# MasterXiong/Hyper-VLA

Measured on AMD Instinct MI355X. Metric: actions_per_sec, higher is better.
Workload: dtype f16; 1 GPU; BASELINE configs[1]: hypernet weight-gen once (untimed) + full sample_actions step (u8 224x224 -> DINOv2-base E=768 in the loop -> generated vit_t 4L/64d policy -> [4,7] action chunk); 1 action = 1 sample-step; batch_per_gpu=256, global_batch=256, encoder=DINOv2-base (reference parity, E=768), parallelism=episode-dp1 (no collectives), policy_operands=split-bf16 (bf16x3), launch=eager (114 launches per step, counted by the library), streams=1, ensemble=not in the step

## Files before the change

### hyper-vla_amd/csrc/api.hip

```cpp
#include <hip/hip_runtime.h>

#include <cmath>
#include <cstdio>
#include <cstring>
#include <map>
#include <memory>
#include <mutex>
#include <string>
#include <vector>

#include "../../include/hvla.h"
#include "common.h"
#include "kernels.h"
#include "layout.h"
#include "pack.h"
#include "serving_layout.h"
#include "t5.h"
#include "train.h"

using namespace hvla;

namespace {

struct DevBuf {
// ... 1058 lines not shown
  return HVLA_OK;
}

int hvla_profile_read(hvla_ctx* ctx, float* ms, int32_t* launches) {
  if (!ctx || !ms || !launches) return HVLA_E_STATE;
  HIPCHK(ctx, hipSetDevice(ctx->device));
  for (int i = 0; i < HVLA_PROF_N; ++i) ms[i] = 0.f, launches[i] = 0;
  Profiler& p = ctx->prof;
  for (size_t i = 0; i < p.used; ++i) {
    HIPCHK(ctx, hipEventSynchronize(p.stop[i]));
    float t = 0.f;
    HIPCHK(ctx, hipEventElapsedTime(&t, p.start[i], p.stop[i]));
    ms[p.cat[i]] += t;
    launches[p.cat[i]] += 1;
  }
  p.used = 0;
  return HVLA_OK;
}

#ifdef HVLA_BENCH_HOOKS
int hvla_debug_gemm(hvla_ctx* ctx, int M, int N, int K, int epi, int variant, int iters, float* ms) {
  if (!ctx || !ctx->loaded) return HVLA_E_STATE;
  HIPCHK(ctx, hipSetDevice(ctx->device));
  const void* A = ctx->ws[K > ctx->g.E ? WS_G : WS_H].p;
  void* out = ctx->ws[epi == 3 ? WS_X : (epi == 1 ? WS_QKV : WS_G)].p;
  if (epi == 2 && K > ctx->g.E) return HVLA_E_SHAPE;
  const EncLayerW& L = ctx->encw.layer[0];
  const void* W = epi == 1 ? L.wqkv : (epi == 2 ? L.w1 : (K > ctx->g.E ? L.w2 : L.wo));
  const float* bias = epi == 1 ? L.bqkv : (epi == 2 ? L.b1 : L.b2);
  HIPCHK(ctx, debug_gemm(A, W, bias, L.ls1, out, M, N, K, epi, variant, iters, ms, nullptr));
  return HVLA_OK;
}

int hvla_debug_bgemm(const float* A, const float* B, float* C, int M, int N, int K, int ta, int tb, int nb, int accumulate,
                     int iters, float* ms) {
  const int lda = ta ? M : K, ldb = tb ? K : N;
  BG g{A, B, C, nullptr, M, N, K, lda, ldb, N, (long)M * K, 0, (long)N * K, 0, (long)M * N, 0, 0, 1, 1.f, accumulate, 1, accumulate != 0};
  hipEvent_t e0, e1;
  (void)hipEventCreate(&e0);
  (void)hipEventCreate(&e1);
  for (int i = 0; i < 3; ++i) bgemm(nullptr, ta != 0, tb != 0, g, nb);
  (void)hipEventRecord(e0, nullptr);
  for (int i = 0; i < iters; ++i) bgemm(nullptr, ta != 0, tb != 0, g, nb);
  (void)hipEventRecord(e1, nullptr);
  (void)hipEventSynchronize(e1);
  (void)hipEventElapsedTime(ms, e0, e1);
  *ms /= iters;
  (void)hipEventDestroy(e0);
  (void)hipEventDestroy(e1);
  return hipGetLastError() == hipSuccess ? HVLA_OK : HVLA_E_HIP;
}

struct hvla_bgemm_desc {
  const float* A;
  const float* B;
  float* C;
  const float* bias;
  int32_t M, N, K, lda, ldb, ldc;
  int64_t sA0, sA1, sB0, sB1, sC0, sC1, sBias0, sBias1;
  int32_t nb1;
  float alpha;
  int32_t accumulate, ksplit, allow_split, a_padded;
  int32_t ta, tb, nb0;
};
int hvla_debug_bgemm_once(const hvla_bgemm_desc* d, int32_t* chosen) {
  if (!d || !chosen || d->nb0 < 1 || d->nb1 < 1 || d->ksplit < 1 || d->M < 1 || d->N < 1 || d->K < 1) return (int)hipErrorInvalidValue;
// ... 110 lines not shown
```

### hyper-vla_amd/csrc/encoder.hip

```cpp
#include <cstring>
#include <type_traits>

#include "common.h"
#include "kernels.h"
#include "plan.h"

namespace hvla {

template <typename Op>
__global__ void im2col_kernel(const uint8_t* __restrict__ img, typename Op::elem* __restrict__ out, int B,
                              int image, int patch, int grid, int Kp, float* __restrict__ x, const float* __restrict__ pos, int S, int E) {
  for (size_t i = (size_t)blockIdx.x * blockDim.x + threadIdx.x; i < (size_t)B * E; i += (size_t)gridDim.x * blockDim.x)
    x[(i / E) * S * E + (i % E)] = pos[i % E];
  const int Kp1 = Kp / 2, chunks = Kp1 / 8;
  const size_t total = (size_t)B * grid * grid * chunks;
  const int kreal = patch * patch * 3;
  for (size_t i = (size_t)blockIdx.x * blockDim.x + threadIdx.x; i < total; i += (size_t)gridDim.x * blockDim.x) {
    const int ch = (int)(i % chunks);
    const size_t m = i / chunks;
    const int px = (int)(m % grid), py = (int)((m / grid) % grid);
    const size_t b = m / ((size_t)grid * grid);
    typename Op::x8 v;
    const int rowb = 3 * patch;
    const int k0 = ch * 8;
// ... 25 lines not shown
  const void* abar2 = nullptr;
  const void* dW2 = nullptr;
  float* corr2 = nullptr;
  int M2 = 0;
  int row0 = 0, row_step = 1;
  int hsplit = 1 << 30;
  int tile_row0 = 0, tile_stride = 256, nbm = 0;
  void* colmean = nullptr;
  void* ln_out = nullptr;
  const float* ln_scale = nullptr;
  const float* ln_bias = nullptr;
  void* ln_abar = nullptr;
  uint32_t* ln_cnt = nullptr;
  float* ln_part = nullptr;
  uint32_t ln_target = 0;
  uint32_t ln_tag = 0;
  uint32_t ln_spin = 0;
  uint32_t out_bytes = 0;
  uint32_t part_bytes = 0;
  int lnx_G = 0, lnx_rows_aligned = 0, lnx_rounds_div = 0, lnx_rows_xcd = 0, lnx_rcp = 0;
  const float* ln_partial = nullptr;
};

__device__ __forceinline__ int wperm(int rho) { return (rho & ~63) + 4 * (rho & 15) + ((rho >> 4) & 3); }
__device__ __forceinline__ f32x4 corr_value(f32x4 acc, float b) {
  return f32x4{fmaf(acc[0], 1.f / 4096.f, b), fmaf(acc[1], 1.f / 4096.f, b), fmaf(acc[2], 1.f / 4096.f, b), fmaf(acc[3], 1.f / 4096.f, b)};
}

template <typename Op, int EPI, int MT, bool FULL, bool ROWBIAS, bool CS = false, bool WT = false, bool NT = false>
__device__ __forceinline__ void gemm_epilogue_rows_impl(const f32x4 (&acc)[4][MT], const GemmArgs& g, int m_base, int n_base,
                                                        int fr, int fq, const f32x4* pre_b4, const f32x4* pre_l4,
                                                        typename Op::x4* cs = nullptr,
                                                        const __attribute__((address_space(3))) float* lds_corr = nullptr,
                                                        int lds_img0 = -1) {
  using T = typename Op::elem;
  const int n = n_base + 4 * fr;
  f32x4 b4 = f32x4{0.f, 0.f, 0.f, 0.f};
  if constexpr (!ROWBIAS) b4 = pre_b4 ? *pre_b4 : *reinterpret_cast<const f32x4*>(g.bias + n);
  f32x4 l4 = f32x4{1.f, 1.f, 1.f, 1.f};
  if constexpr (EPI == EPI_RES) l4 = pre_l4 ? *pre_l4 : *reinterpret_cast<const f32x4*>(g.aux + n);
  const float q = EPI == EPI_PATCH ? g.qscale : ((EPI == EPI_QKV && n_base < g.qcols) ? g.qscale : 1.f);
  __amdgpu_buffer_rsrc_t wt_rsrc;
  if constexpr (WT) wt_rsrc = __builtin_amdgcn_make_buffer_rsrc(g.out, 0, (int)g.out_bytes, 0x00020000);
  auto store_f32x4 = [&](uint32_t elem_off, f32x4 v) {
    if constexpr (WT) __builtin_amdgcn_raw_buffer_store_b128(__builtin_bit_cast(u32x4, v), wt_rsrc, (int)(elem_off * 4u), 0, 16);
    else *reinterpret_cast<f32x4*>(reinterpret_cast<float*>(g.out) + elem_off) = v;
  };
  __amdgpu_buffer_rsrc_t nt_rsrc;
  uint32_t nt_vo = 0;
  if constexpr (NT && FULL && (EPI == EPI_QKV || EPI == EPI_GELU)) {
    nt_rsrc = __builtin_amdgcn_make_buffer_rsrc(g.out, 0, -1, 0x00020000);
    nt_vo = ((uint32_t)(g.row0 + (m_base + 4 * fq) * g.row_step) * (uint32_t)g.N + (uint32_t)n) * (uint32_t)sizeof(T);
  }
  constexpr int RB = MT < 2 ? 1 : (EPI == EPI_RES && MT >= 4 ? 4 : 2);
#pragma unroll
  for (int mp = 0; mp < MT; mp += RB) {
    f32x4 xin[RB][4], brow[RB][4];
    uint32_t off[RB][4];
    bool ok[RB][4];
#pragma unroll
    for (int u = 0; u < RB; ++u)
#pragma unroll
      for (int r = 0; r < 4; ++r) {
        const int m = m_base + (mp + u) * 16 + 4 * fq + r;
        ok[u][r] = FULL || m < g.M;
        const int grow = g.row0 + m * g.row_step;
        off[u][r] = (uint32_t)grow * (uint32_t)g.N + (uint32_t)n;
        if constexpr (EPI == EPI_PATCH) {
          const int prow = 1 + (m % g.P);
          off[u][r] = (uint32_t)((m / g.P) * g.S + prow) * (uint32_t)g.N + (uint32_t)n;
          if (ok[u][r]) xin[u][r] = *reinterpret_cast<const f32x4*>(g.aux + (uint32_t)prow * (uint32_t)g.N + (uint32_t)n);
        }
        if constexpr (EPI == EPI_RES) {
          if (ok[u][r]) {
            if constexpr (NT) xin[u][r] = __builtin_nontemporal_load(reinterpret_cast<const f32x4*>(reinterpret_cast<const float*>(g.out) + off[u][r]));
            else xin[u][r] = *reinterpret_cast<const f32x4*>(reinterpret_cast<const float*>(g.out) + off[u][r]);
          }
        }
        if constexpr (ROWBIAS) {
          brow[u][r] = f32x4{0.f, 0.f, 0.f, 0.f};
          const int img = grow / g.S;
          const int tok = grow - img * g.S, hf = tok >= g.hsplit ? 1 : 0;
          if (lds_img0 >= 0) {
            if (ok[u][r]) {
              if (tok) brow[u][r] = *reinterpret_cast<const __attribute__((address_space(3))) f32x4*>(lds_corr + ((img - lds_img0) * 2 + hf) * 64 + 4 * fr);
              else brow[u][r] = *reinterpret_cast<const f32x4*>(g.bias + (uint32_t)n);
            }
          } else {
            const float* bsrc = tok ? g.corr + (uint32_t)(img * 2 + hf) * (uint32_t)g.N : g.bias;
            if (ok[u][r]) brow[u][r] = *reinterpret_cast<const f32x4*>(bsrc + (uint32_t)n);
          }
        }
      }
#pragma unroll
    for (int u = 0; u < RB; ++u) {
      f32x4 t[4];
#pragma unroll
      for (int c = 0; c < 4; ++c) {
        if constexpr (EPI == EPI_PATCH) t[c] = __builtin_elementwise_fma(acc[c][mp + u], f32x4{q, q, q, q}, f32x4{b4[c], b4[c], b4[c], b4[c]});
        else if constexpr (EPI == EPI_CORR) t[c] = corr_value(acc[c][mp + u], b4[c]);
        else if constexpr (ROWBIAS) t[c] = acc[c][mp + u] + f32x4{brow[u][0][c], brow[u][1][c], brow[u][2][c], brow[u][3][c]};
        else t[c] = acc[c][mp + u] + b4[c];
        if constexpr (EPI == EPI_QKV) t[c] *= q;
        if constexpr (EPI == EPI_GELU) {
          const f32x2 g0 = gelu_erf2(f32x2{t[c][0], t[c][1]}), g1 = gelu_erf2(f32x2{t[c][2], t[c][3]});
          t[c] = f32x4{g0[0], g0[1], g1[0], g1[1]};
        }
// ... 2 lines not shown
      for (int r = 0; r < 4; ++r) {
        if (!ok[u][r]) continue;
        if constexpr (EPI == EPI_QKV || EPI == EPI_GELU) {
          typename Op::x4 o;
#pragma unroll
          for (int c = 0; c < 4; ++c) o[c] = (T)t[c][r];
          if constexpr (CS) *cs += o;
          if constexpr (NT && FULL) {
            int rowb = g.row_step * g.N * (int)sizeof(T);
            asm volatile("" : "+s"(rowb));
            __builtin_amdgcn_raw_buffer_store_b64(__builtin_bit_cast(u32x2, o), nt_rsrc, (int)nt_vo, ((mp + u) * 16 + r) * rowb, 2);
          } else if constexpr (NT) __builtin_nontemporal_store(o, reinterpret_cast<typename Op::x4*>(reinterpret_cast<T*>(g.out) + off[u][r]));
          else *reinterpret_cast<typename Op::x4*>(reinterpret_cast<T*>(g.out) + off[u][r]) = o;
        } else if constexpr (EPI == EPI_RES) {
          f32x4 x = xin[u][r];
#pragma unroll
          for (int c = 0; c < 4; ++c) x[c] = fmaf(t[c][r], l4[c], x[c]);
          store_f32x4(off[u][r], x);
        } else if constexpr (EPI == EPI_CORR) {
          *reinterpret_cast<f32x4*>(reinterpret_cast<float*>(g.out) + off[u][r]) = f32x4{t[0][r], t[1][r], t[2][r], t[3][r]};
        } else {
          f32x4 x = xin[u][r];
#pragma unroll
          for (int c = 0; c < 4; ++c) x[c] += t[c][r];
          store_f32x4(off[u][r], x);
        }
      }
    }
  }
}

template <typename Op, int EPI, int MT>
__device__ __forceinline__ void gemm_epilogue_rows(const f32x4 (&acc)[4][MT], const GemmArgs& g, int m_base, int n_base,
                                                   int fr, int fq) {
  const bool full = m_base + 16 * MT <= g.M;
  if constexpr (EPI == EPI_PATCH || EPI == EPI_CORR) {
    if (full) gemm_epilogue_rows_impl<Op, EPI, MT, true, false>(acc, g, m_base, n_base, fr, fq, nullptr, nullptr);
    else gemm_epilogue_rows_impl<Op, EPI, MT, false, false>(acc, g, m_base, n_base, fr, fq, nullptr, nullptr);
  } else {
    if (g.corr) {
      if (full) gemm_epilogue_rows_impl<Op, EPI, MT, true, true>(acc, g, m_base, n_base, fr, fq, nullptr, nullptr);
      else gemm_epilogue_rows_impl<Op, EPI, MT, false, true>(acc, g, m_base, n_base, fr, fq, nullptr, nullptr);
    } else {
      if (full) gemm_epilogue_rows_impl<Op, EPI, MT, true, false>(acc, g, m_base, n_base, fr, fq, nullptr, nullptr);
      else gemm_epilogue_rows_impl<Op, EPI, MT, false, false>(acc, g, m_base, n_base, fr, fq, nullptr, nullptr);
    }
  }
}


template <typename Op, int EPI>
__global__ __launch_bounds__(256, 2) void gemm_kernel(GemmArgs g) {
  using T = typename Op::elem;
  using X8 = typename Op::x8;
  extern __shared__ __attribute__((aligned(16))) char smem[];
  T* As = reinterpret_cast<T*>(smem);
  T* Ws = As + 2 * GBM * GLD;
  const int tid = threadIdx.x, wave = tid >> 6, lane = tid & 63;
  const int wm = wave >> 1, wn = wave & 1;
  const int nbm = (g.M + GBM - 1) / GBM, nbn = g.N / GBN;
  const int bid = xcd_run(blockIdx.x, nbm * nbn);
  const int bm = bid % nbm, bn = bid / nbm;
  const int m0 = bm * GBM, n0 = bn * GBN;
  const T* A = reinterpret_cast<const T*>(g.A);
  const T* W = reinterpret_cast<const T*>(g.W);

  const int lrow = tid >> 3, lch = tid & 7;
  const T* ap[4];
  const T* wp[4];
#pragma unroll
  for (int i = 0; i < 4; ++i) {
    int m = m0 + lrow + 32 * i;
    m = m < g.M ? m : g.M - 1;
    ap[i] = A + (size_t)(g.row0 + m * g.row_step) * g.K + lch * 8;
    wp[i] = W + (size_t)(n0 + wperm(lrow + 32 * i)) * g.K + lch * 8;
  }
  X8 ra[4], rw[4];
  auto gload = [&](int kt) {
// ... 28 lines not shown
    const T* as = As + (buf * GBM + wm * 64 + fr) * GLD + fq * 8;
    const T* ws = Ws + (buf * GBN + wn * 64 + fr) * GLD + fq * 8;
#pragma unroll
    for (int kk = 0; kk < 2; ++kk) {
      X8 fa[4], fw[4];
#pragma unroll
      for (int t = 0; t < 4; ++t) {
        fa[t] = *reinterpret_cast<const X8*>(as + t * 16 * GLD + kk * 32);
        fw[t] = *reinterpret_cast<const X8*>(ws + t * 16 * GLD + kk * 32);
      }
#pragma unroll
      for (int nt = 0; nt < 4; ++nt)
#pragma unroll
        for (int mt = 0; mt < 4; ++mt) acc[nt][mt] = Op::mma16(fa[mt], fw[nt], acc[nt][mt]);
    }
    if (kt + 1 < KT) sstore(buf ^ 1);
    __syncthreads();
  }

  gemm_epilogue_rows<Op, EPI, 4>(acc, g, m0 + wm * 64, n0 + wn * 64, fr, fq);
}

template <typename Op, int EPI, int NS = SNS>
__device__ __forceinline__ void gemm64_body(const GemmArgs& g, int bm, int bn) {
  using T = typename Op::elem;
  using X8 = typename Op::x8;
  extern __shared__ __attribute__((aligned(16))) char smem[];
  const int tid = threadIdx.x, lane = tid & 63;
  const int wave = __builtin_amdgcn_readfirstlane(tid >> 6);
  const int m0 = bm * SBM, n0 = bn * SBN;
  const T* A = reinterpret_cast<const T*>(g.A);
  const T* W = reinterpret_cast<const T*>(g.W);
  const int sch = ((lane & 7) ^ (lane >> 3)) * 8;
  uint32_t aoff[2], woff[2];
#pragma unroll
  for (int j = 0; j < 2; ++j) {
    const int rl = 32 * j + 8 * wave + (lane >> 3);
    int m = m0 + rl;
    m = m < g.M ? m : g.M - 1;
    aoff[j] = (uint32_t)(g.row0 + m * g.row_step) * (uint32_t)g.K + sch;
    woff[j] = (uint32_t)(n0 + wperm(rl)) * (uint32_t)g.K + sch;
  }
  const int KT = g.K / 64;
  auto issue = [&](int kt) {
    char* base = smem + (kt % NS) * 16384 + wave * 1024;
#pragma unroll
    for (int j = 0; j < 2; ++j) {
      __builtin_amdgcn_global_load_lds((const __attribute__((address_space(1))) void*)(A + aoff[j] + kt * 64),
                                       (__attribute__((address_space(3))) void*)(base + j * 4096), 16, 0, 0);
      __builtin_amdgcn_global_load_lds((const __attribute__((address_space(1))) void*)(W + woff[j] + kt * 64),
                                       (__attribute__((address_space(3))) void*)(base + 8192 + j * 4096), 16, 0, 0);
    }
  };
  f32x4 acc[4][1];
#pragma unroll
  for (int i = 0; i < 4; ++i) acc[i][0] = f32x4{0.f, 0.f, 0.f, 0.f};
  const int fr = lane & 15, fq = lane >> 4;
  const int sw0 = (fq ^ (fr & 7)) << 4, sw1 = ((fq + 4) ^ (fr & 7)) << 4;
  const int a_off = (wave * 16 + fr) * 128, w_off = 8192 + fr * 128;
#pragma unroll
  for (int s = 0; s < NS - 1; ++s)
    if (s < KT) issue(s);
  for (int kt = 0; kt < KT; ++kt) {
    const int issued = kt + NS - 1 < KT ? kt + NS - 1 : KT;
    switch (issued - kt - 1) {
      case 0: asm volatile("s_waitcnt vmcnt(0)" ::: "memory"); break;
      case 1: asm volatile("s_waitcnt vmcnt(4)" ::: "memory"); break;
      case 2: asm volatile("s_waitcnt vmcnt(8)" ::: "memory"); break;
      case 3: asm volatile("s_waitcnt vmcnt(12)" ::: "memory"); break;
      default: asm volatile("s_waitcnt vmcnt(16)" ::: "memory"); break;
    }
    __builtin_amdgcn_sched_barrier(0);
    __builtin_amdgcn_s_barrier();
    asm volatile("" ::: "memory");
    __builtin_amdgcn_sched_barrier(0);
    const char* lb = smem + (kt % NS) * 16384;
    X8 fa[2], fw[4][2];
    fa[0] = *reinterpret_cast<const X8*>(lb + a_off + sw0);
    fa[1] = *reinterpret_cast<const X8*>(lb + a_off + sw1);
#pragma unroll
    for (int nt = 0; nt < 4; ++nt) {
      fw[nt][0] = *reinterpret_cast<const X8*>(lb + w_off + nt * 2048 + sw0);
      fw[nt][1] = *reinterpret_cast<const X8*>(lb + w_off + nt * 2048 + sw1);
    }
    __builtin_amdgcn_sched_barrier(0);
    if (kt + NS - 1 < KT) issue(kt + NS - 1);
    asm volatile("s_waitcnt lgkmcnt(0)" ::: "memory");
    __builtin_amdgcn_sched_barrier(0);
#pragma unroll
    for (int kk = 0; kk < 2; ++kk)
#pragma unroll
      for (int nt = 0; nt < 4; ++nt) acc[nt][0] = Op::mma16(fa[kk], fw[nt][kk], acc[nt][0]);
  }
  gemm_epilogue_rows<Op, EPI, 1>(acc, g, m0 + wave * 16, n0, fr, fq);
}

template <typename Op, int EPI, int NS = SNS>
__global__ __launch_bounds__(256) void gemm64_kernel(GemmArgs g) {
  const int nbm1 = (g.M + SBM - 1) / SBM, nbm2 = (g.M2 + SBM - 1) / SBM, rt_all = nbm1 + nbm2;
  const int t = xcd_run(blockIdx.x, gridDim.x);
  const int bn = t / rt_all, bm = t - bn * rt_all;
  if (bm < nbm1) {
    gemm64_body<Op, EPI, NS>(g, bm, bn);
  } else {
    GemmArgs c = g;
    c.A = g.abar2; c.W = g.dW2; c.out = g.corr2; c.M = g.M2; c.row0 = 0; c.row_step = 1; c.corr = nullptr;
    gemm64_body<Op, EPI_CORR, NS>(c, bm - nbm1, bn);
  }
}

__device__ __forceinline__ f32x4 ln_half_sum(const f32x4* p, int n4) { return (p[0] + p[n4]) + (p[2 * n4] + p[3 * n4]); }
template <typename Op, int EPI, bool FOLD = false>
__global__ __launch_bounds__(256) void gemm64c_kernel(GemmArgs g) {
  constexpr int SST = FOLD ? SSTF : SSTC, PCS = FOLD ? 6 : 7;
  using T = typename Op::elem;
  using X8 = typename Op::x8;
  extern __shared__ __attribute__((aligned(16))) char smem[];
  const int tid = threadIdx.x, lane = tid & 63;
  const int wave = __builtin_amdgcn_readfirstlane(tid >> 6);
  const int nbm = (g.M + SBM - 1) / SBM;
  const int tix = xcd_run(blockIdx.x, gridDim.x), bm = tix % nbm, bn = tix / nbm;
  const int m0 = bm * SBM, n0 = bn * SBN;
  const T* A = reinterpret_cast<const T*>(g.A);
  const T* W = reinterpret_cast<const T*>(g.W);
  const T* dW = reinterpret_cast<const T*>(g.dW2);
  const T* AB = reinterpret_cast<const T*>(g.abar2);
  const int img0 = (g.row0 + m0 * g.row_step) / g.S;
  const int sch = ((lane & 7) ^ (lane >> 3)) * 8;
  uint32_t aoff[2], woff[2], boff;
#pragma unroll
  for (int j = 0; j < 2; ++j) {
    const int rl = 32 * j + 8 * wave + (lane >> 3);
    int m = m0 + rl;
    m = m < g.M ? m : g.M - 1;
// ... 1731 lines not shown
    HVLA_STOP_HERE();
  }
#undef HVLA_STOP_HERE
  pf.begin(call.final_norm.cat, st);
  if (keep_cls)
    HVLA_LAUNCH((layernorm_kernel<Op, 2>), grid_of(call.final_norm), dim3(call.final_norm.block), 0, st, ws.x, tokens, w.lnf_s, w.lnf_b, M, E, S);
  else
    HVLA_LAUNCH((layernorm_kernel<Op, 1>), grid_of(call.final_norm), dim3(call.final_norm.block), 0, st, ws.x, tokens, w.lnf_s, w.lnf_b, M, E, S);
  pf.end(call.final_norm.cat, st);
  return hipGetLastError();
}

#undef HVLA_LAUNCH
#ifdef HVLA_BENCH_HOOKS
hipError_t debug_lnx_stats(unsigned long long* out, int reset) {
  hipError_t e = hipDeviceSynchronize();
  if (e == hipSuccess && out) e = hipMemcpyFromSymbol(out, HIP_SYMBOL(g_lnx_dbg), sizeof(unsigned long long) * 8 * 256);
  if (e == hipSuccess && reset) {
    static unsigned long long zero[8][256];
    e = hipMemcpyToSymbol(HIP_SYMBOL(g_lnx_dbg), zero, sizeof zero);
  }
  return e;
}
hipError_t debug_gemm(const void* A, const void* W, const float* bias, const float* aux, void* out, int M, int N,
                      int K, int epi, int variant, int iters, float* ms, hipStream_t st) {
  using Op = OpF16;
  GemmArgs a{A, W, M, N, K, bias, aux, out, 256, 257, epi == EPI_QKV ? N / 3 : 0, 0.125f};
  a.nbm = M / HBM_; a.tile_row0 = 0; a.tile_stride = HBM_;
  if (epi < EPI_QKV || epi > EPI_RES || variant < 0 || variant > 3 || N % HBN_ || K % 64 || (variant >= 2 && a.nbm < 1)) return hipErrorInvalidValue;
  int ncu = 256;
  (void)device_setup<Op>(ncu);
  const int nt = a.nbm * (N / HBN_);
  const Launch forms[4] = {{G128_PATCH + epi, (unsigned)(((M + GBM - 1) / GBM) * (N / GBN)), 1, 256, (size_t)2 * (GBM + GBN) * GLD * 2},
                           {G64_PATCH + epi, (unsigned)(((M + SBM - 1) / SBM) * (N / SBN)), 1, 256, (size_t)SNS * SST},
                           {G256_PATCH + 2 * epi, (unsigned)nt, 1, 512, P256_LDS},
                           {G256_PATCH + 2 * epi + 1, (unsigned)(nt < ncu ? nt : ncu), 1, 512, P256_LDS}};
  const Launch& f = forms[variant];
  auto launch = [&]() { hipLaunchKernelGGL(EncKernels<Op>::gemm()[f.kernel], grid_of(f), dim3(f.block), f.lds, st, a); };
  hipEvent_t e0, e1;
  (void)hipEventCreate(&e0);
  (void)hipEventCreate(&e1);
  launch();
  (void)hipEventRecord(e0, st);
  for (int i = 0; i < iters; ++i) launch();
  (void)hipEventRecord(e1, st);
  (void)hipEventSynchronize(e1);
  (void)hipEventElapsedTime(ms, e0, e1);
  *ms /= iters;
  (void)hipEventDestroy(e0);
  (void)hipEventDestroy(e1);
  return hipGetLastError();
}
hipError_t debug_attention_stamps(const void* qkv, void* o, void* omean, int B, int S, int E, int H, int wg, unsigned long long* stamps,
                                  hipStream_t st) {
  using Op = OpF16;
  using T = Op::elem;
  int ncu = 256;
  (void)device_setup<Op>(ncu);
  const Launch at = plan_attention(B, S, H, sizeof(T), false);
  hipLaunchKernelGGL(EncKernels<Op>::attn()[at.kernel], grid_of(at), dim3(at.block), at.lds, st, reinterpret_cast<const T*>(qkv),
                     reinterpret_cast<T*>(o), S, E, H, reinterpret_cast<T*>(omean), (float*)nullptr, 0, stamps, wg);
  return hipGetLastError();
}
#endif

hipError_t launch_encoder(const Geom& g, int dtype, const EncWeights& w, const EncWorkspace& ws,
                          const uint8_t* images, float* tokens, int B, hipStream_t st, Profiler* prof, bool keep_cls,
                          uint32_t* audit) {
  if (dtype == 1) return run_encoder<OpBF16>(g, w, ws, images, tokens, B, st, prof, keep_cls, audit);
  return run_encoder<OpF16>(g, w, ws, images, tokens, B, st, prof, keep_cls, audit);
}

}
```

### hyper-vla_amd/csrc/kernels.h

```cpp
#pragma once
#include <hip/hip_runtime.h>
#include <stdint.h>

#include <vector>

#include "../../include/hvla.h"
#include "accept.h"
#include "layout.h"

namespace hvla {

struct CtxLayer {
  const float *ln0_s, *ln0_b, *wq, *bq, *wk, *bk, *wv, *bv, *wo, *bo, *ln1_s, *ln1_b, *w1, *b1, *w2, *b2;
};
struct CtxParams {
  int T, C, F, heads, layers, lang_dim, E, scale_context;
  int big_elems;
  const float* tok;
  const int64_t* attn_mask;
  const float* cls;
  const float *w_tok, *b_tok, *w_img, *b_img, *pos_tok, *pos_img, *pos_layer, *norm_s, *norm_b;
  CtxLayer layer[CTX_MAX_LAYERS];
  float* ctx;
  __bf16 *ctx_hi, *ctx_lo;
// ... 47 lines not shown
  int stop_after = 0;
#endif
};
struct Profiler {
  int mode = 0;
  uint32_t select = 1u << 5;
  std::vector<hipEvent_t> start, stop;
  std::vector<int> cat;
  size_t used = 0;
  uint64_t nlaunch = 0;
  bool want(int c) const { return c >= 0 && (mode == 2 || (mode == 1 && ((select >> c) & 1u))); }
  void begin(int c, hipStream_t st) {
    if (!want(c)) return;
    if (used == start.size()) {
      hipEvent_t a, b;
      if (hipEventCreate(&a) != hipSuccess || hipEventCreate(&b) != hipSuccess) return;
      start.push_back(a), stop.push_back(b), cat.push_back(c);
    }
    cat[used] = c;
    (void)hipEventRecord(start[used], st);
  }
  void end(int c, hipStream_t st) {
    if (!want(c) || used >= start.size()) return;
    (void)hipEventRecord(stop[used], st);
    ++used;
  }
};
hipError_t launch_encoder(const Geom& g, int dtype, const EncWeights& w, const EncWorkspace& ws,
                          const uint8_t* images, float* tokens, int B, hipStream_t st, Profiler* prof,
                          bool keep_cls = false,
                          uint32_t* audit = nullptr);

#ifdef HVLA_BENCH_HOOKS
hipError_t debug_gemm(const void* A, const void* W, const float* bias, const float* aux, void* out, int M, int N,
                      int K, int epi, int variant, int iters, float* ms, hipStream_t st);
hipError_t debug_lnx_stats(unsigned long long* out, int reset);
hipError_t debug_ctx_stamps(unsigned long long* out);
hipError_t debug_attention_stamps(const void* qkv, void* o, void* omean, int B, int S, int E, int H, int wg, unsigned long long* stamps,
                                  hipStream_t st);
#endif

void build_resize_spans(int in_size, int out_size, std::vector<int>& start, std::vector<int>& count, std::vector<float>& w,
                        int& maxspan);
hipError_t launch_resize(const uint8_t* src, uint8_t* dst, float* tmp_rows, float* tmp_img, const int* row_start,
                         const int* row_count, const float* row_w, int row_span, const int* col_start, const int* col_count,
                         const float* col_w, int col_span, int B, int H, int W, int S, int crop, hipStream_t st,
                         float* padded = nullptr, int src_h = 0, int src_w = 0);

struct PolicyParams {
  PolicyLayout pl;
  const __bf16 *wh, *wl;
  const float* vf;
  const float* tokens;
  float* actions;
  float* logits;
  int B, E, P, L, M, horizon, action_dim;
  float tanh_scale, max_action;
  float* amap = nullptr;
#ifdef HVLA_BENCH_HOOKS
  unsigned long long* stamps = nullptr;
#endif
};
hipError_t launch_policy(const PolicyParams& p, hipStream_t st, int lang_T = 0, const int32_t* slots = nullptr, int rows = 0);
struct LangPrefixParams {
  PolicyLayout pl;
  int m_lproj, m_lkv, v_lproj_b, v_lpos;
  __bf16 *wh, *wl;
  const float* vf;
// ... 54 lines not shown
```

### hyper-vla_amd/csrc/plan.h

```cpp
#pragma once
#include <stddef.h>
#include <stdint.h>

#ifdef __HIPCC__
#define HVLA_HD __host__ __device__ __forceinline__
#else
#define HVLA_HD inline
#endif

namespace hvla {

HVLA_HD int xcd_run(int bid, int nwg) {
  const int q = nwg / 8, r = nwg % 8, xcd = bid % 8;
  return (xcd < r ? xcd * (q + 1) : r * (q + 1) + (xcd - r) * q) + bid / 8;
}

HVLA_HD bool big_output(size_t rows, size_t cols, size_t elem_bytes) { return rows * cols * elem_bytes >= ((size_t)96 << 20); }

HVLA_HD bool nt16_addressable(size_t rows, size_t cols, size_t elem_bytes) { return rows * cols * elem_bytes < ((size_t)1 << 32); }

enum { EPI_PATCH = 0, EPI_QKV = 1, EPI_GELU = 2, EPI_RES = 3, EPI_CORR = 4 };
constexpr int GBM = 128, GBN = 128, GBK = 64, GLD = 72;
constexpr int SBM = 64, SBN = 64, SNS = 6, SST = 16384;
constexpr int SNSC = 5, SSTC = 28672;
// ... 30 lines not shown
  X(G256NT_GELU, gemm256p_kernel<Op, EPI_GELU, false, false, true>) X(G256NT_GELU_P, gemm256p_kernel<Op, EPI_GELU, true, false, true>) \
  X(G256NT_RES, gemm256p_kernel<Op, EPI_RES, false, false, true>) X(G256NT_RES_P, gemm256p_kernel<Op, EPI_RES, true, false, true>) \
  X(G256LN_PATCH, gemm256p_kernel<Op, EPI_PATCH, false, true>) X(G256LN_PATCH_P, gemm256p_kernel<Op, EPI_PATCH, true, true>) \
  X(G256LN_RES, gemm256p_kernel<Op, EPI_RES, false, true>) X(G256LN_RES_P, gemm256p_kernel<Op, EPI_RES, true, true>) \
  X(G256LNNT_RES, gemm256p_kernel<Op, EPI_RES, false, true, true>) X(G256LNNT_RES_P, gemm256p_kernel<Op, EPI_RES, true, true, true>)
enum GemmKernel : int {
#define HVLA_X(id, ...) id,
  HVLA_GEMM_KERNELS(HVLA_X)
#undef HVLA_X
  NUM_GEMM_KERNELS
};
static_assert(G128_PATCH + EPI_RES == G128_RES && G64_PATCH + EPI_CORR == G64_CORR && G64S4_QKV - EPI_QKV + EPI_RES == G64S4_RES, "");
static_assert(G64C_QKV - EPI_QKV + EPI_RES == G64C_RES && G64CF_QKV - EPI_QKV + EPI_GELU == G64CF_GELU, "");
static_assert(G256_PATCH + 2 * EPI_RES + 1 == G256_RES_P && G256NT_QKV + 2 * (EPI_RES - EPI_QKV) + 1 == G256NT_RES_P, "");
static_assert(G256LN_PATCH + 1 == G256LN_PATCH_P && G256LN_RES + 1 == G256LN_RES_P && G256LNNT_RES + 1 == G256LNNT_RES_P, "");
enum AttnKernel : int { ATT, ATT_U, ATT_MAP, NUM_ATTN_KERNELS };
enum OtherKernel : int { IM2COL = 100, LN_GROUP, LN_MEAN, COLMEAN, LN_FINAL };

struct Launch {
  int kernel = -1;
  unsigned grid = 0, grid_y = 1, block = 0;
  size_t lds = 0;
  int cat = -1;
  explicit operator bool() const { return kernel >= 0; }
};
struct EncSizes {
  int B, P, S, E, F, H, patch, layers;
  int ncu;
  size_t elem;
  bool comp, ln_ws, amap;
  int M() const { return B * S; }
};
HVLA_HD int ceil_div(int a, int b) { return (a + b - 1) / b; }

constexpr int LNX_MAX_E = 1024;
constexpr int LNX_TILES = LNX_MAX_E / HBN_;
constexpr int LNX_ENTRY_BYTES = 16, LNX_CNT_ALIGN = 16;
static_assert(LNX_TILES == 4 && LNX_MAX_E % HBN_ == 0, "");
inline size_t lnx_cnt_bytes(int nb) { return ((size_t)nb * sizeof(uint32_t) + LNX_CNT_ALIGN - 1) / LNX_CNT_ALIGN * LNX_CNT_ALIGN; }
inline size_t lnx_part_bytes(int nb, int E) { return (size_t)nb * ((E + HBN_ - 1) / HBN_) * HBM_ * LNX_ENTRY_BYTES; }

inline bool small_fused(const EncSizes& z, int N, int K) {
  return z.comp && z.M() <= G64_MAXM && (size_t)z.M() * K < (1ull << 31) && (size_t)N * K < (1ull << 31) && N % SBN == 0 && K % 64 == 0 && z.S >= 9;
}
inline bool can_fuse_ln(const EncSizes& z) { return z.ln_ws && (size_t)z.M() * z.E * 4 < (1ull << 32) && z.E <= LNX_MAX_E; }
inline bool lnx_persistent(int ncu, int nbm, int nbn) {
  const int nt = nbm * nbn;
  if (ncu % 8 || nt % ncu || nbm % 8) return false;
  const int Wx = ncu / 8, odd = Wx % nbn, R = nt / ncu;
  return Wx >= nbn && (odd == 0 || R % nbn == 0);
}

struct GemmPlan {
  Launch small;
  Launch main;
  bool aligned = false;
  bool fused_bias = false;
  bool fold = false;
  bool ln_fused = false;
  int tile_row0 = 0, tile_stride = 256, nbm = 0, nbn = 0;
  int lnx_G = 0, lnx_rows_aligned = 0, lnx_rounds_div = 0, lnx_rows_xcd = 0, lnx_rcp = 0;
};
inline void plan_lnx(const EncSizes& z, GemmPlan& p, int base) {
  const bool persist = lnx_persistent(z.ncu, p.nbm, p.nbn);
  p.main.kernel = base + persist;
  p.main.grid = persist ? z.ncu : p.nbm * p.nbn;
  p.ln_fused = true;
  if (persist) {
    const int Wx = z.ncu / 8, R = p.nbm * p.nbn / z.ncu;
    p.lnx_G = Wx / p.nbn; p.lnx_rows_aligned = R * p.lnx_G; p.lnx_rounds_div = R / p.nbn; p.lnx_rows_xcd = p.nbm / 8;
    p.lnx_rcp = (65536 + p.nbn - 1) / p.nbn;
  }
}
inline GemmPlan plan_gemm(const EncSizes& z, int epi, int N, int K, int cat, bool ln_follows, bool ln_partial) {
  GemmPlan p;
  const int B = z.B, ncu = z.ncu, M = epi == EPI_PATCH ? B * z.P : z.M();
  const bool fits32 = (size_t)M * K < (1ull << 31) && (epi == EPI_PATCH || (size_t)N * K < (1ull << 31));
  p.main.block = 256;
  p.main.cat = cat;
  p.nbn = ceil_div(N, HBN_);
  p.aligned = N % SBN == 0 && N >= HBN_ && M > G64_MAXM && fits32 &&
              (epi == EPI_PATCH ? M % HBM_ == 0 : z.P == HBM_ && K >= 128 && K % 64 == 0);
  if (p.aligned) {
    p.main.block = 512;
    p.main.lds = P256_LDS;
    if (epi == EPI_PATCH) {
      p.nbm = M / HBM_; p.tile_row0 = 0; p.tile_stride = HBM_;
      if (z.P == HBM_ && can_fuse_ln(z) && ln_follows) { plan_lnx(z, p, G256LN_PATCH); return p; }
    } else {
      int nblocks = ceil_div(B, SBM) * (N / SBN);
      if (z.comp) nblocks += ceil_div(2 * B, SBM) * (N / SBN);
      const bool two_per_cu = nblocks > ncu;
      p.small = Launch{two_per_cu ? G64S4_QKV - EPI_QKV + epi : G64_PATCH + epi, (unsigned)nblocks, 1, 256, (size_t)(two_per_cu ? 4 : SNS) * SST, CAT_COMP};
      p.nbm = B; p.tile_row0 = 1; p.tile_stride = z.S;
      if (epi == EPI_RES && ln_follows && can_fuse_ln(z)) {
        plan_lnx(z, p, big_output(M, N, sizeof(float)) ? G256LNNT_RES : G256LN_RES);
        return p;
      }
      if (big_output(M, N, epi == EPI_RES ? sizeof(float) : z.elem) && (epi == EPI_RES || nt16_addressable(M, N, z.elem))) {
        const bool persist = (B * p.nbn) % ncu == 0;
        p.main.kernel = G256NT_QKV + 2 * (epi - EPI_QKV) + persist;
        p.main.grid = persist ? ncu : B * p.nbn;
        return p;
      }
    }
    const bool persist = (p.nbm * p.nbn) % ncu == 0;
    p.main.kernel = G256_PATCH + 2 * epi + persist;
    p.main.grid = persist ? ncu : p.nbm * p.nbn;
    return p;
  }
  if (epi != EPI_PATCH && small_fused(z, N, K)) {
    const int nb64 = ceil_div(M, SBM) * (N / SBN);
    p.fused_bias = true;
    if (epi != EPI_RES && ln_partial) {
      p.fold = true;
      p.main.kernel = G64CF_QKV - EPI_QKV + epi; p.main.grid = nb64; p.main.lds = gemm64c_fold_lds(K);
    } else if (epi == EPI_RES && 2 * nb64 <= ncu) {
      p.main.kernel = G64C32; p.main.grid = 2 * nb64; p.main.lds = (size_t)SNS32 * SST32;
    } else {
      p.main.kernel = G64C_QKV - EPI_QKV + epi; p.main.grid = nb64; p.main.lds = (size_t)SNSC * SSTC;
    }
    return p;
  }
  if (epi != EPI_PATCH && z.comp)
    p.small = Launch{G64_CORR, (unsigned)(ceil_div(2 * B, SBM) * (N / SBN)), 1, 256, (size_t)SNS * SST, CAT_COMP};
  if (M <= G64_MAXM && fits32 && N % SBN == 0 && (epi == EPI_PATCH || K % 64 == 0)) {
    p.main.kernel = G64_PATCH + epi; p.main.grid = ceil_div(M, SBM) * (N / SBN); p.main.lds = (size_t)SNS * SST;
  } else {
    p.main.kernel = G128_PATCH + epi; p.main.grid = ceil_div(M, GBM) * (N / GBN); p.main.lds = (size_t)2 * (GBM + GBN) * GLD * z.elem;
  }
  return p;
}

struct NormPlan {
  Launch group, mean;
  bool partial = false, fold = false;
};
inline NormPlan plan_norm(const EncSizes& z, int Nnext, int scratch_cols) {
  NormPlan n;
  n.group = Launch{LN_GROUP, LNG, (unsigned)z.B, LNW * 64, (size_t)(z.P / 8) * z.E * sizeof(float), 1};
  n.partial = z.comp && (size_t)LNG * z.E * sizeof(float) <= (size_t)z.S * scratch_cols * z.elem;
  n.fold = n.partial && small_fused(z, Nnext, z.E) && gemm64c_fold_lds(z.E) <= LDS_LIMIT && ceil_div(z.M(), SBM) * (Nnext / SBN) <= z.ncu;
  if (n.partial && !n.fold) n.mean = Launch{LN_MEAN, 2u * z.B, 1, 256, 0, 1};
  return n;
}

inline Launch plan_attention(int B, int S, int H, size_t elem, bool amap) {
  const int KT = (S + 31) / 32;
  return Launch{amap ? ATT_MAP : KT == 9 ? ATT_U : ATT, (unsigned)(B * H), 1, (unsigned)(KT - 1) * 64, attention_lds(KT, elem, amap), 3};
}

struct CallPlan {
  bool ok = false;
  int Kp = 0;
  size_t cnt_bytes = 0, part_bytes = 0;
  Launch im2col, attention, colmean, final_norm;
};
inline CallPlan plan_call(const EncSizes& z) {
  CallPlan c;
  const int M = z.M();
// ... 37 lines not shown
```

Before: 18380 actions/s.

## Rework gemm64 k-loop with inline-asm LDS loads and prefetched epilogue operands

The 64-wide GEMM body now issues its global-to-LDS loads through inline assembly that sets m0 explicitly and uses buffer-relative offsets. The k-loop is split into a steady-state part with a fixed vmcnt wait and a drain part. The per-tile lgkmcnt(0) wait is dropped, and bias, layer-scale and residual inputs are loaded before the main loop, so the epilogue no longer waits on fresh global reads. It also adds a grid helper, an out-of-range block guard, and a debug probe entry point. The gains come at the cost of fragile hand-written asm with manual m0 handling, and higher register pressure from the prefetched operands.

New measurement: 18430 actions/s (median of 6 runs). No clear change (+0.3%).

```diff
diff --git a/hyper-vla_amd/csrc/api.hip b/hyper-vla_amd/csrc/api.hip
--- a/hyper-vla_amd/csrc/api.hip
+++ b/hyper-vla_amd/csrc/api.hip
@@ -1114,6 +1114,21 @@
   return HVLA_OK;
 }
 
+int hvla_debug_gemm64_grid(hvla_ctx* ctx, int M, int N, int K, int M2_args, int M2_grid, size_t out_offset) {
+  if (!ctx || !ctx->loaded) return HVLA_E_STATE;
+  HIPCHK(ctx, hipSetDevice(ctx->device));
+  const EncLayerW& L = ctx->encw.layer[0];
+  const int M2 = M2_args > M2_grid ? M2_args : M2_grid;
+  if (M < 1 || N < 64 || N % 64 || N > 3 * ctx->g.E || K < 64 || K % 64 || K > ctx->g.E || M2_args < 0 || M2_grid < 0 || out_offset % 16 ||
+      (size_t)M * K * 2 > ctx->ws[WS_H].bytes || out_offset + (size_t)M * N * 2 > ctx->ws[WS_QKV].bytes ||
+      (size_t)M2 * K * 2 > ctx->ws[WS_ABAR].bytes || (size_t)M2 * N * 4 > ctx->ws[WS_CORR].bytes || !L.dqkv)
+    return HVLA_E_SHAPE;
+  GemmArgs64Probe q{ctx->ws[WS_H].p, L.wqkv, ctx->ws[WS_ABAR].p, L.dqkv, L.bqkv, (char*)ctx->ws[WS_QKV].p + out_offset,
+                    (float*)ctx->ws[WS_CORR].p, M, N, K, M2_args, M2_grid};
+  HIPCHK(ctx, debug_gemm64_grid(q, nullptr));
+  HIPCHK(ctx, hipDeviceSynchronize());
+  return HVLA_OK;
+}
 int hvla_debug_bgemm(const float* A, const float* B, float* C, int M, int N, int K, int ta, int tb, int nb, int accumulate,
                      int iters, float* ms) {
   const int lda = ta ? M : K, ldb = tb ? K : N;
diff --git a/hyper-vla_amd/csrc/encoder.hip b/hyper-vla_amd/csrc/encoder.hip
--- a/hyper-vla_amd/csrc/encoder.hip
+++ b/hyper-vla_amd/csrc/encoder.hip
@@ -81,7 +81,8 @@
                                                         int fr, int fq, const f32x4* pre_b4, const f32x4* pre_l4,
                                                         typename Op::x4* cs = nullptr,
                                                         const __attribute__((address_space(3))) float* lds_corr = nullptr,
-                                                        int lds_img0 = -1) {
+                                                        int lds_img0 = -1,
+                                                        const f32x4* pre_x = nullptr) {
   using T = typename Op::elem;
   const int n = n_base + 4 * fr;
   f32x4 b4 = f32x4{0.f, 0.f, 0.f, 0.f};
@@ -121,7 +122,9 @@
           if (ok[u][r]) xin[u][r] = *reinterpret_cast<const f32x4*>(g.aux + (uint32_t)prow * (uint32_t)g.N + (uint32_t)n);
         }
         if constexpr (EPI == EPI_RES) {
-          if (ok[u][r]) {
+          if (pre_x) {
+            xin[u][r] = pre_x[(mp + u) * 4 + r];
+          } else if (ok[u][r]) {
             if constexpr (NT) xin[u][r] = __builtin_nontemporal_load(reinterpret_cast<const f32x4*>(reinterpret_cast<const float*>(g.out) + off[u][r]));
             else xin[u][r] = *reinterpret_cast<const f32x4*>(reinterpret_cast<const float*>(g.out) + off[u][r]);
           }
@@ -190,18 +193,19 @@
 
 template <typename Op, int EPI, int MT>
 __device__ __forceinline__ void gemm_epilogue_rows(const f32x4 (&acc)[4][MT], const GemmArgs& g, int m_base, int n_base,
-                                                   int fr, int fq) {
+                                                   int fr, int fq, const f32x4* pre_b4 = nullptr, const f32x4* pre_l4 = nullptr,
+                                                   const f32x4* pre_x = nullptr) {
   const bool full = m_base + 16 * MT <= g.M;
   if constexpr (EPI == EPI_PATCH || EPI == EPI_CORR) {
-    if (full) gemm_epilogue_rows_impl<Op, EPI, MT, true, false>(acc, g, m_base, n_base, fr, fq, nullptr, nullptr);
-    else gemm_epilogue_rows_impl<Op, EPI, MT, false, false>(acc, g, m_base, n_base, fr, fq, nullptr, nullptr);
+    if (full) gemm_epilogue_rows_impl<Op, EPI, MT, true, false>(acc, g, m_base, n_base, fr, fq, pre_b4, nullptr);
+    else gemm_epilogue_rows_impl<Op, EPI, MT, false, false>(acc, g, m_base, n_base, fr, fq, pre_b4, nullptr);
   } else {
     if (g.corr) {
-      if (full) gemm_epilogue_rows_impl<Op, EPI, MT, true, true>(acc, g, m_base, n_base, fr, fq, nullptr, nullptr);
-      else gemm_epilogue_rows_impl<Op, EPI, MT, false, true>(acc, g, m_base, n_base, fr, fq, nullptr, nullptr);
+      if (full) gemm_epilogue_rows_impl<Op, EPI, MT, true, true>(acc, g, m_base, n_base, fr, fq, nullptr, pre_l4, nullptr, nullptr, -1, pre_x);
+      else gemm_epilogue_rows_impl<Op, EPI, MT, false, true>(acc, g, m_base, n_base, fr, fq, nullptr, pre_l4, nullptr, nullptr, -1, pre_x);
     } else {
-      if (full) gemm_epilogue_rows_impl<Op, EPI, MT, true, false>(acc, g, m_base, n_base, fr, fq, nullptr, nullptr);
-      else gemm_epilogue_rows_impl<Op, EPI, MT, false, false>(acc, g, m_base, n_base, fr, fq, nullptr, nullptr);
+      if (full) gemm_epilogue_rows_impl<Op, EPI, MT, true, false>(acc, g, m_base, n_base, fr, fq, pre_b4, pre_l4, nullptr, nullptr, -1, pre_x);
+      else gemm_epilogue_rows_impl<Op, EPI, MT, false, false>(acc, g, m_base, n_base, fr, fq, pre_b4, pre_l4, nullptr, nullptr, -1, pre_x);
     }
   }
 }
@@ -296,25 +300,44 @@
   const T* A = reinterpret_cast<const T*>(g.A);
   const T* W = reinterpret_cast<const T*>(g.W);
   const int sch = ((lane & 7) ^ (lane >> 3)) * 8;
-  uint32_t aoff[2], woff[2];
+  uint32_t avo[2], wvo[2];
 #pragma unroll
   for (int j = 0; j < 2; ++j) {
     const int rl = 32 * j + 8 * wave + (lane >> 3);
     int m = m0 + rl;
     m = m < g.M ? m : g.M - 1;
-    aoff[j] = (uint32_t)(g.row0 + m * g.row_step) * (uint32_t)g.K + sch;
-    woff[j] = (uint32_t)(n0 + wperm(rl)) * (uint32_t)g.K + sch;
+    avo[j] = ((uint32_t)(g.row0 + m * g.row_step) * (uint32_t)g.K + sch) * (uint32_t)sizeof(T);
+    wvo[j] = ((uint32_t)(n0 + wperm(rl)) * (uint32_t)g.K + sch) * (uint32_t)sizeof(T);
   }
   const int KT = g.K / 64;
-  auto issue = [&](int kt) {
-    char* base = smem + (kt % NS) * 16384 + wave * 1024;
-#pragma unroll
-    for (int j = 0; j < 2; ++j) {
-      __builtin_amdgcn_global_load_lds((const __attribute__((address_space(1))) void*)(A + aoff[j] + kt * 64),
-                                       (__attribute__((address_space(3))) void*)(base + j * 4096), 16, 0, 0);
-      __builtin_amdgcn_global_load_lds((const __attribute__((address_space(1))) void*)(W + woff[j] + kt * 64),
-                                       (__attribute__((address_space(3))) void*)(base + 8192 + j * 4096), 16, 0, 0);
-    }
+  __builtin_amdgcn_s_waitcnt(0x0F70);
+  const int fr_ = lane & 15, fq_ = lane >> 4;
+  f32x4 pb4 = f32x4{0.f, 0.f, 0.f, 0.f}, pl4 = pb4, px[4] = {pb4, pb4, pb4, pb4};
+  if constexpr (EPI != EPI_PATCH) {
+    pb4 = *reinterpret_cast<const f32x4*>(g.bias + n0 + 4 * fr_);
+    if constexpr (EPI == EPI_RES) {
+      pl4 = *reinterpret_cast<const f32x4*>(g.aux + n0 + 4 * fr_);
+#pragma unroll
+      for (int r = 0; r < 4; ++r) {
+        int m = m0 + wave * 16 + 4 * fq_ + r;
+        m = m < g.M ? m : g.M - 1;
+        px[r] = *reinterpret_cast<const f32x4*>(reinterpret_cast<const float*>(g.out) + ((uint32_t)(g.row0 + m * g.row_step) * (uint32_t)g.N + (uint32_t)(n0 + 4 * fr_)));
+      }
+    }
+  }
+  const uint32_t lds0 = (uint32_t)(uintptr_t)(__attribute__((address_space(3))) char*)smem + (uint32_t)wave * 1024u;
+  auto issue = [&](int kt, uint32_t stage) {
+    const uint32_t dst = lds0 + stage;
+    const T* ab = A + kt * 64;
+    const T* wb = W + kt * 64;
+    uint32_t keep;
+    asm volatile("s_mov_b32 %0, m0\n\t"
+                 "s_mov_b32 m0, %7\n\ts_nop 0\n\tglobal_load_lds_dwordx4 %1, %5\n\t"
+                 "s_add_u32 m0, %7, 0x1000\n\ts_nop 0\n\tglobal_load_lds_dwordx4 %2, %5\n\t"
+                 "s_add_u32 m0, %7, 0x2000\n\ts_nop 0\n\tglobal_load_lds_dwordx4 %3, %6\n\t"
+                 "s_add_u32 m0, %7, 0x3000\n\ts_nop 0\n\tglobal_load_lds_dwordx4 %4, %6\n\t"
+                 "s_mov_b32 m0, %0"
+                 : "=&s"(keep) : "v"(avo[0]), "v"(avo[1]), "v"(wvo[0]), "v"(wvo[1]), "s"(ab), "s"(wb), "s"(dst) : "scc");
   };
   f32x4 acc[4][1];
 #pragma unroll
@@ -324,39 +347,49 @@
   const int a_off = (wave * 16 + fr) * 128, w_off = 8192 + fr * 128;
 #pragma unroll
   for (int s = 0; s < NS - 1; ++s)
-    if (s < KT) issue(s);
-  for (int kt = 0; kt < KT; ++kt) {
-    const int issued = kt + NS - 1 < KT ? kt + NS - 1 : KT;
-    switch (issued - kt - 1) {
+    if (s < KT) issue(s, (uint32_t)s * 16384u);
+  uint32_t rd = 0, wr = (uint32_t)(NS - 1) * 16384u;
+  auto tile = [&](int kt, auto do_issue) {
+    __builtin_amdgcn_sched_barrier(0);
+    __builtin_amdgcn_s_barrier();
+    asm volatile("" ::: "memory");
+    __builtin_amdgcn_sched_barrier(0);
+    const char* lb = smem + rd;
+    X8 fa[2], fw[4][2];
+    fa[0] = *reinterpret_cast<const X8*>(lb + a_off + sw0);
+    fa[1] = *reinterpret_cast<const X8*>(lb + a_off + sw1);
+#pragma unroll
+    for (int nt = 0; nt < 4; ++nt) {
+      fw[nt][0] = *reinterpret_cast<const X8*>(lb + w_off + nt * 2048 + sw0);
+      fw[nt][1] = *reinterpret_cast<const X8*>(lb + w_off + nt * 2048 + sw1);
+    }
+    __builtin_amdgcn_sched_barrier(0);
+    if constexpr (decltype(do_issue)::value) issue(kt + NS - 1, wr);
+    __builtin_amdgcn_sched_barrier(0);
+#pragma unroll
+    for (int kk = 0; kk < 2; ++kk)
+#pragma unroll
+      for (int nt = 0; nt < 4; ++nt) acc[nt][0] = Op::mma16(fa[kk], fw[nt][kk], acc[nt][0]);
+    wr = rd;
+    rd = rd + 16384u == (uint32_t)NS * 16384u ? 0u : rd + 16384u;
+  };
+  int kt = 0;
+  for (; kt + NS - 1 < KT; ++kt) {
+    asm volatile("s_waitcnt vmcnt(%0)" ::"n"(4 * (NS - 2)) : "memory");
+    tile(kt, std::true_type{});
+  }
+  for (; kt < KT; ++kt) {
+    switch (KT - kt - 1) {
       case 0: asm volatile("s_waitcnt vmcnt(0)" ::: "memory"); break;
       case 1: asm volatile("s_waitcnt vmcnt(4)" ::: "memory"); break;
       case 2: asm volatile("s_waitcnt vmcnt(8)" ::: "memory"); break;
       case 3: asm volatile("s_waitcnt vmcnt(12)" ::: "memory"); break;
       default: asm volatile("s_waitcnt vmcnt(16)" ::: "memory"); break;
     }
-    __builtin_amdgcn_sched_barrier(0);
-    __builtin_amdgcn_s_barrier();
-    asm volatile("" ::: "memory");
-    __builtin_amdgcn_sched_barrier(0);
-    const char* lb = smem + (kt % NS) * 16384;
-    X8 fa[2], fw[4][2];
-    fa[0] = *reinterpret_cast<const X8*>(lb + a_off + sw0);
-    fa[1] = *reinterpret_cast<const X8*>(lb + a_off + sw1);
-#pragma unroll
-    for (int nt = 0; nt < 4; ++nt) {
-      fw[nt][0] = *reinterpret_cast<const X8*>(lb + w_off + nt * 2048 + sw0);
-      fw[nt][1] = *reinterpret_cast<const X8*>(lb + w_off + nt * 2048 + sw1);
-    }
-    __builtin_amdgcn_sched_barrier(0);
-    if (kt + NS - 1 < KT) issue(kt + NS - 1);
-    asm volatile("s_waitcnt lgkmcnt(0)" ::: "memory");
-    __builtin_amdgcn_sched_barrier(0);
-#pragma unroll
-    for (int kk = 0; kk < 2; ++kk)
-#pragma unroll
-      for (int nt = 0; nt < 4; ++nt) acc[nt][0] = Op::mma16(fa[kk], fw[nt][kk], acc[nt][0]);
-  }
-  gemm_epilogue_rows<Op, EPI, 1>(acc, g, m0 + wave * 16, n0, fr, fq);
+    tile(kt, std::false_type{});
+  }
+  if constexpr (EPI == EPI_PATCH) gemm_epilogue_rows<Op, EPI, 1>(acc, g, m0 + wave * 16, n0, fr, fq);
+  else gemm_epilogue_rows<Op, EPI, 1>(acc, g, m0 + wave * 16, n0, fr, fq, &pb4, &pl4, EPI == EPI_RES ? px : nullptr);
 }
 
 template <typename Op, int EPI, int NS = SNS>
@@ -364,6 +397,7 @@
   const int nbm1 = (g.M + SBM - 1) / SBM, nbm2 = (g.M2 + SBM - 1) / SBM, rt_all = nbm1 + nbm2;
   const int t = xcd_run(blockIdx.x, gridDim.x);
   const int bn = t / rt_all, bm = t - bn * rt_all;
+  if (bn >= g.N / SBN) return;
   if (bm < nbm1) {
     gemm64_body<Op, EPI, NS>(g, bm, bn);
   } else {
@@ -2161,7 +2195,7 @@
   (void)device_setup<Op>(ncu);
   const int nt = a.nbm * (N / HBN_);
   const Launch forms[4] = {{G128_PATCH + epi, (unsigned)(((M + GBM - 1) / GBM) * (N / GBN)), 1, 256, (size_t)2 * (GBM + GBN) * GLD * 2},
-                           {G64_PATCH + epi, (unsigned)(((M + SBM - 1) / SBM) * (N / SBN)), 1, 256, (size_t)SNS * SST},
+                           {G64_PATCH + epi, gemm64_grid(M, 0, N), 1, 256, (size_t)SNS * SST},
                            {G256_PATCH + 2 * epi, (unsigned)nt, 1, 512, P256_LDS},
                            {G256_PATCH + 2 * epi + 1, (unsigned)(nt < ncu ? nt : ncu), 1, 512, P256_LDS}};
   const Launch& f = forms[variant];
@@ -2180,6 +2214,17 @@
   (void)hipEventDestroy(e1);
   return hipGetLastError();
 }
+hipError_t debug_gemm64_grid(const GemmArgs64Probe& q, hipStream_t st) {
+  using Op = OpF16;
+  if (q.N % SBN || q.K % 64 || q.M < 1 || q.M2_args < 0 || q.M2_grid < 0) return hipErrorInvalidValue;
+  GemmArgs a{q.A, q.W, q.M, q.N, q.K, q.bias, nullptr, q.out, 256, 257, q.N / 3, 0.125f};
+  if (q.M2_args > 0) { a.abar2 = q.abar2; a.dW2 = q.dW2; a.corr2 = q.corr2; a.M2 = q.M2_args; }
+  int ncu = 256;
+  (void)device_setup<Op>(ncu);
+  const Launch f{G64_QKV, gemm64_grid(q.M, q.M2_grid, q.N), 1, 256, (size_t)SNS * SST};
+  hipLaunchKernelGGL(EncKernels<Op>::gemm()[f.kernel], grid_of(f), dim3(f.block), f.lds, st, a);
+  return hipGetLastError();
+}
 hipError_t debug_attention_stamps(const void* qkv, void* o, void* omean, int B, int S, int E, int H, int wg, unsigned long long* stamps,
                                   hipStream_t st) {
   using Op = OpF16;
diff --git a/hyper-vla_amd/csrc/kernels.h b/hyper-vla_amd/csrc/kernels.h
--- a/hyper-vla_amd/csrc/kernels.h
+++ b/hyper-vla_amd/csrc/kernels.h
@@ -103,8 +103,16 @@
                           uint32_t* audit = nullptr);
 
 #ifdef HVLA_BENCH_HOOKS
+struct GemmArgs64Probe {
+  const void *A, *W, *abar2, *dW2;
+  const float* bias;
+  void* out;
+  float* corr2;
+  int M, N, K, M2_args, M2_grid;
+};
 hipError_t debug_gemm(const void* A, const void* W, const float* bias, const float* aux, void* out, int M, int N,
                       int K, int epi, int variant, int iters, float* ms, hipStream_t st);
+hipError_t debug_gemm64_grid(const GemmArgs64Probe& q, hipStream_t st);
 hipError_t debug_lnx_stats(unsigned long long* out, int reset);
 hipError_t debug_ctx_stamps(unsigned long long* out);
 hipError_t debug_attention_stamps(const void* qkv, void* o, void* omean, int B, int S, int E, int H, int wg, unsigned long long* stamps,
diff --git a/hyper-vla_amd/csrc/plan.h b/hyper-vla_amd/csrc/plan.h
--- a/hyper-vla_amd/csrc/plan.h
+++ b/hyper-vla_amd/csrc/plan.h
@@ -86,6 +86,7 @@
   int M() const { return B * S; }
 };
 HVLA_HD int ceil_div(int a, int b) { return (a + b - 1) / b; }
+HVLA_HD unsigned gemm64_grid(int M, int M2, int N) { return (unsigned)((ceil_div(M, SBM) + ceil_div(M2, SBM)) * (N / SBN)); }
 
 constexpr int LNX_MAX_E = 1024;
 constexpr int LNX_TILES = LNX_MAX_E / HBN_;
@@ -142,8 +143,7 @@
       p.nbm = M / HBM_; p.tile_row0 = 0; p.tile_stride = HBM_;
       if (z.P == HBM_ && can_fuse_ln(z) && ln_follows) { plan_lnx(z, p, G256LN_PATCH); return p; }
     } else {
-      int nblocks = ceil_div(B, SBM) * (N / SBN);
-      if (z.comp) nblocks += ceil_div(2 * B, SBM) * (N / SBN);
+      const int nblocks = (int)gemm64_grid(B, z.comp ? 2 * B : 0, N);
       const bool two_per_cu = nblocks > ncu;
       p.small = Launch{two_per_cu ? G64S4_QKV - EPI_QKV + epi : G64_PATCH + epi, (unsigned)nblocks, 1, 256, (size_t)(two_per_cu ? 4 : SNS) * SST, CAT_COMP};
       p.nbm = B; p.tile_row0 = 1; p.tile_stride = z.S;
@@ -177,9 +177,9 @@
     return p;
   }
   if (epi != EPI_PATCH && z.comp)
-    p.small = Launch{G64_CORR, (unsigned)(ceil_div(2 * B, SBM) * (N / SBN)), 1, 256, (size_t)SNS * SST, CAT_COMP};
+    p.small = Launch{G64_CORR, gemm64_grid(2 * B, 0, N), 1, 256, (size_t)SNS * SST, CAT_COMP};
   if (M <= G64_MAXM && fits32 && N % SBN == 0 && (epi == EPI_PATCH || K % 64 == 0)) {
-    p.main.kernel = G64_PATCH + epi; p.main.grid = ceil_div(M, SBM) * (N / SBN); p.main.lds = (size_t)SNS * SST;
+    p.main.kernel = G64_PATCH + epi; p.main.grid = gemm64_grid(M, 0, N); p.main.lds = (size_t)SNS * SST;
   } else {
     p.main.kernel = G128_PATCH + epi; p.main.grid = ceil_div(M, GBM) * (N / GBN); p.main.lds = (size_t)2 * (GBM + GBN) * GLD * z.elem;
   }
```
